# vilnik/incorporating-different-sources

Hardware: AMD Instinct MI355X
Metric: rolling windows/sec (higher is better)
Workload: dtype f64

## Files before the change

### incorporating_different_sources_amd/csrc/posterior_wave_impl.h

```cpp
#pragma once
#include <utility>

#include "posterior_fused_impl.h"

namespace {

template <int NT_, bool LEAN_ = true>
struct WCfg {
    static constexpr int NT = NT_;
    static constexpr int KP = 16 * NT;
    static constexpr int NTILES = NT * (NT + 1) / 2;
    static constexpr int MLD = 17;
    static constexpr int OFF_M = 0;
    static constexpr int OFF_DG = OFF_M + NT * 16 * MLD;
    static constexpr int OFF_IDT = OFF_DG + 256;
    static constexpr int OFF_VEC = OFF_IDT + 256;
    static constexpr int LDS_DOUBLES = OFF_VEC + KP;
    static constexpr int LDS_BYTES = LDS_DOUBLES * 8;
    static constexpr int OFF_SUB = LDS_DOUBLES;
};
constexpr int WAVE_LDS_LIMIT = 64 * 1024;
__host__ __device__ inline int wave_idx_rows(int n_r, int m, bool conj) {
    const int r = (conj && m > n_r) ? m : n_r;
    return (r + 63) & ~63;
}
__host__ __device__ inline int wave_idx_bytes(int n_r, int m, bool conj) { return wave_idx_rows(n_r, m, conj) * 12; }

constexpr int wtile(int NT, int I, int J) { return I * NT - I * (I - 1) / 2 + (J - I); }

template <int I, int J>
__device__ __forceinline__ void wave_post_tile(double* P, int k, int fr, int fq, const d4& t) {
    const int gj = 16 * J + fr;
#pragma unroll
    for (int r = 0; r < 4; ++r) {
        const int gi = 16 * I + fq + 4 * r;
        if (gi < k && gj < k && (I < J || gi <= gj)) {
            tp_post_store(P + (long long)gi * k + gj, t[r]);
            if (I < J || gi < gj) tp_post_store(P + (long long)gj * k + gi, t[r]);
        }
    }
}

template <int NT, int NWV>
constexpr int w2_owner(int J) {
    const int p = NT - 1 - J, g = p / NWV, i = p % NWV;
    return (g & 1) ? NWV - 1 - i : i;
}
template <int NT, int NWV>
constexpr int w2_count(int WV) {
    int n = 0;
    for (int J = 0; J < NT; ++J)
        if (w2_owner<NT, NWV>(J) == WV) n += J + 1;
    return n;
}
template <int NT, int NWV>
constexpr int w2_max_tiles() {
    int m = 0;
    for (int w = 0; w < NWV; ++w) m = w2_count<NT, NWV>(w) > m ? w2_count<NT, NWV>(w) : m;
    return m;
}
template <int NT, int NWV>
constexpr int w2_slot(int I, int J) {
    const int wv = w2_owner<NT, NWV>(J);
    int n = 0;
    for (int i = 0; i < NT; ++i)
        for (int j = i; j < NT; ++j) {
            if (i == I && j == J) return n;
            if (w2_owner<NT, NWV>(j) == wv) ++n;
        }
    return -1;
}
template <int NT, int NWV>
constexpr bool w2_owns_from(int WV, int I) {
    for (int J = I; J < NT; ++J)
        if (w2_owner<NT, NWV>(J) == WV) return true;
    return false;
}
template <int NT>
constexpr bool w2_one_wave_is_whole() {
    for (int J = 0; J < NT; ++J) {
        if (w2_owner<NT, 1>(J) != 0) return false;
        for (int I = 0; I <= J; ++I)
            if (w2_slot<NT, 1>(I, J) != wtile(NT, I, J)) return false;
    }
    return w2_count<NT, 1>(0) == NT * (NT + 1) / 2;
}
template <int... N>
constexpr bool w2_one_wave_is_whole_all(std::integer_sequence<int, N...>) { return (w2_one_wave_is_whole<N + 1>() && ...); }
static_assert(w2_one_wave_is_whole_all(std::make_integer_sequence<int, 15>{}),
              "w2_owner<NT,1>(J) == 0, w2_slot<NT,1>(I,J) == wtile(NT,I,J), w2_count<NT,1>(0) == NT(NT+1)/2 for NT = 1..15");

constexpr bool wave_tile_in_agpr(int t) { return t < 32; }

template <int T>
__device__ __forceinline__ void wave_mfma_agpr(d4& c, double a, double b) {
    if constexpr (wave_tile_in_agpr(T)) asm volatile("s_nop 1\n\tv_mfma_f64_16x16x4_f64 %0, %1, %2, %0" : "+a"(c) : "v"(a), "v"(b));
    else asm volatile("s_nop 1\n\tv_mfma_f64_16x16x4_f64 %0, %1, %2, %0" : "+v"(c) : "v"(a), "v"(b));
}
template <int T>
__device__ __forceinline__ void wave_settle1(d4& c0) {
    if constexpr (wave_tile_in_agpr(T)) asm volatile("s_nop 15\n\ts_nop 7" : "+a"(c0));
    else asm volatile("s_nop 15\n\ts_nop 7" : "+v"(c0));
}
template <int T>
__device__ __forceinline__ void wave_pin1(d4& c0) {
    if constexpr (wave_tile_in_agpr(T)) asm volatile("" : "+a"(c0));
    else asm volatile("" : "+v"(c0));
}
__device__ __forceinline__ void wave_settle14(d4& c0, d4& c1, d4& c2, d4& c3, d4& c4, d4& c5, d4& c6, d4& c7, d4& c8, d4& c9,
                                              d4& c10, d4& c11, d4& c12, d4& c13) {
    asm volatile("s_nop 15\n\ts_nop 7" : "+a"(c0), "+a"(c1), "+a"(c2), "+a"(c3), "+a"(c4), "+a"(c5), "+a"(c6), "+a"(c7), "+a"(c8),
                 "+a"(c9), "+a"(c10), "+a"(c11), "+a"(c12), "+a"(c13));
}
template <int N>
__device__ __forceinline__ void wave_pin(d4 (&acc)[N]) {
    static_for<0, N>([&](auto tc) __attribute__((always_inline)) { wave_pin1<decltype(tc)::value>(acc[decltype(tc)::value]); });
}
template <bool GROUPED, int N>
__device__ __forceinline__ void wave_settle(d4 (&acc)[N]) {
    if constexpr (GROUPED) {
        static_for<0, (N + 13) / 14>([&](auto gc) __attribute__((always_inline)) {
            constexpr int b = 14 * decltype(gc)::value;
            if constexpr (b + 14 <= N && wave_tile_in_agpr(b + 13)) {
                wave_settle14(acc[b], acc[b + 1], acc[b + 2], acc[b + 3], acc[b + 4], acc[b + 5], acc[b + 6], acc[b + 7], acc[b + 8],
                              acc[b + 9], acc[b + 10], acc[b + 11], acc[b + 12], acc[b + 13]);
            } else {
                static_for<b, (b + 14 < N ? b + 14 : N)>([&](auto tc) __attribute__((always_inline)) {
                    wave_settle1<decltype(tc)::value>(acc[decltype(tc)::value]);
                });
            }
        });
    } else {
        wave_settle1<0>(acc[0]);
        static_for<1, N>([&](auto tc) __attribute__((always_inline)) { wave_pin1<decltype(tc)::value>(acc[decltype(tc)::value]); });
    }
}

struct WRows {
    const double* base;
    long long ld;
    const int* ridx;
    long long first;
    const double* sub_row;
    int count;
    int count0;
    int jump;
    bool off32 = false;
};

template <int NT, int NWV, int WV, bool HF, bool LEAN>
__device__ __forceinline__ void wave_gram(const WRows& src, const long long (&coff)[NT], int k, int lane,
                                          double (&shift)[NT], double (&w0v)[NT], bool ones, bool lazy_mask,
                                          d4 (&acc)[w2_count<NT, NWV>(WV)], const int* lds_rows, const double* lds_sub,
                                          double (&csum)[NT], double& usum) {
    constexpr int kI = NT - 1;
    const int fr = lane & 15, fq = lane >> 4;
    const int kc = k - 16 * kI;
    const bool cvl = fr < kc;
    const double border = HF ? ((ones && fr == kc + 1) ? 1.0 : 0.0) : ((fr == kc) ? 1.0 : 0.0);
    const int nks = (src.count + 3) >> 2;
    const bool has_sub = !HF && src.sub_row != nullptr;

    int row_pref = 0;
    double sub_pref = 0.0;
    auto prefetch = [&](int ks) __attribute__((always_inline)) {
        int r = 4 * ks + fq;
        r = r < src.count ? r : src.count - 1;
        row_pref = lds_rows[r];
        if (has_sub) sub_pref = lds_sub[r];
    };
    if constexpr (!LEAN) prefetch(0);
    const char* ub = (const char*)(LEAN ? src.base + src.first * src.ld : src.base);
    const unsigned ld8 = (unsigned)src.ld * 8u;
    unsigned c8[NT];
#pragma unroll
    for (int i = 0; i < NT; ++i) c8[i] = 8u * (unsigned)coff[i];
    auto load = [&](double (&v)[NT], double& sub, int ks) __attribute__((always_inline)) {
        int r = 4 * ks + fq;
        r = r < src.count ? r : src.count - 1;
        if (LEAN || src.off32) {
            unsigned row;
            if constexpr (LEAN) row = (unsigned)(r + (r >= src.count0 ? src.jump : 0));
            else row = (unsigned)row_pref;
            if constexpr (LEAN) {
                const unsigned r0 = __umul24(row, ld8) + c8[0];
#pragma unroll
                for (int i = 0; i < NT - 1; ++i) v[i] = *(const double*)(ub + (size_t)r0 + 128 * i);
                v[NT - 1] = *(const double*)(ub + (size_t)(__umul24(row, ld8) + c8[NT - 1]));
            } else {
                const unsigned ro = __umul24(row, ld8);
#pragma unroll
                for (int i = 0; i < NT; ++i) v[i] = *(const double*)(ub + (size_t)(ro + c8[i]));
            }
        } else {
            const double* p = src.base + (long long)row_pref * src.ld;
#pragma unroll
            for (int i = 0; i < NT; ++i) v[i] = p[coff[i]];
        }
        sub = 0.0;
        if constexpr (!LEAN) {
            if (has_sub) sub = sub_pref;
            prefetch(ks + 1);
        } else {
            if (has_sub) sub = src.sub_row[r];
        }
    };
    auto step = [&](double (&v)[NT], double sub, int ks, auto maskc) __attribute__((always_inline)) {
        constexpr bool MASK = decltype(maskc)::value != 0;
        if (HF) {
#pragma unroll
            for (int i = 0; i < NT; ++i) v[i] -= shift[i];
        } else if (has_sub) {
#pragma unroll
            for (int i = 0; i < NT; ++i) v[i] -= sub;
        }
        v[kI] = cvl ? v[kI] : border;
        if (MASK) {
            const bool rv = 4 * ks + fq < src.count;
#pragma unroll
            for (int i = 0; i < NT; ++i) v[i] = rv ? v[i] : 0.0;
        }
        if (HF) {
            double z = 0.0;
#pragma unroll
            for (int i = 0; i < NT; ++i) z = fma(v[i], w0v[i], z);
            z = rowgroup_sum16(z);
            if (!ones) {
#pragma unroll
                for (int i = 0; i < NT; ++i) csum[i] += v[i];
                usum += z;
            }
            if (fr == kc) v[kI] = z;
        }
        static_for<0, NT>([&](auto Ic) __attribute__((always_inline)) {
            constexpr int I = decltype(Ic)::value;
            static_for<I, NT>([&](auto Jc) __attribute__((always_inline)) {
                constexpr int J = decltype(Jc)::value;
                if constexpr (w2_owner<NT, NWV>(J) == WV) {
                    constexpr int t = w2_slot<NT, NWV>(I, J);
                    wave_mfma_agpr<t>(acc[t], v[I], v[J]);
                }
            });
        });
    };

    if (nks <= 0) return;
    double va[NT], vb[NT], vc[NT];
    double sa = 0.0, sb = 0.0, sc = 0.0;
    load(va, sa, 0);
    load(vb, sb, 1);
    if (HF && lazy_mask) {
        __builtin_amdgcn_sched_barrier(0);
#pragma unroll
        for (int i = 0; i < NT; ++i) {
            const bool cv = 16 * i + fr < k;
            shift[i] = cv ? shift[i] : 0.0;
            w0v[i] = cv ? w0v[i] : 0.0;
        }
    }
    wave_pin(acc);
    int ks = 0;
#pragma nounroll
    for (; 4 * (ks + 3) <= src.count; ks += 3) {
        load(vc, sc, ks + 2);
        step(va, sa, ks, ic<0>{});
        load(va, sa, ks + 3);
        step(vb, sb, ks + 1, ic<0>{});
        load(vb, sb, ks + 4);
        step(vc, sc, ks + 2, ic<0>{});
    }
    if (ks < nks) {
        if (ks + 2 < nks) load(vc, sc, ks + 2);
        step(va, sa, ks, ic<1>{});
        if (ks + 1 < nks) step(vb, sb, ks + 1, ic<1>{});
        if (ks + 2 < nks) step(vc, sc, ks + 2, ic<1>{});
    }
    wave_settle<NWV == 1>(acc);
}

__device__ __forceinline__ void wave_stage_rows(const WRows& src, int lane, int* li, double* lsb) {
    for (int i = lane; i < src.count; i += 64) {
        li[i] = src.ridx ? src.ridx[i] : (int)(src.first + i);
        if (src.sub_row) lsb[i] = src.sub_row[i];
    }
    __builtin_amdgcn_fence(__ATOMIC_RELEASE, "wavefront");
    __builtin_amdgcn_wave_barrier();
}

template <int NT, bool LEAN, int MODE>
__device__ __forceinline__ void wave_window_body(const tp_kargs_t& A, double* lds) {
    constexpr bool FULL = MODE == 2;
    constexpr bool POST = MODE >= 3;
    constexpr int PLAIN = POST ? MODE - 3 : MODE;
    using C = WCfg<NT, LEAN>;
    const int lane = threadIdx.x;
    const int fr = lane & 15, fq = lane >> 4;
    const int k = A.k;
    __builtin_assume(k >= 16 * (NT - 1));
    __builtin_assume(k <= 16 * NT - 1);
    constexpr int kI = NT - 1;
    const int kc = k - 16 * kI;
    const int NTB = (kc == 0) ? NT - 1 : NT;
    const bool colv = fr < kc;
    const long long per_xcd = (A.w_count + 7) >> 3;
    const long long wl = (long long)(blockIdx.x & 7) * per_xcd + (blockIdx.x >> 3);
    if ((long long)(blockIdx.x >> 3) >= per_xcd || wl >= A.w_count) return;
    const long long w = A.w_first + wl;
    const int tid0 = lane;
    (void)tid0;

    const int* cols = (!LEAN && A.col_idx) ? A.col_idx + w * k : nullptr;
    long long coff[NT];
    if (cols != nullptr) {
        int cidx[NT];
#pragma unroll
        for (int i = 0; i < NT; ++i) {
            const int c = 16 * i + fr;
            cidx[i] = cols[c < k ? c : k - 1];
        }
#pragma unroll
        for (int i = 0; i < NT; ++i) coff[i] = (long long)cidx[i];
    } else {
#pragma unroll
        for (int i = 0; i < NT; ++i) {
            const int c = 16 * i + fr;
            coff[i] = (long long)(c < k ? c : k - 1);
        }
    }
    double* idx_sub_lds = LEAN ? nullptr : lds + C::OFF_SUB;
    int* idx_rows_lds = LEAN ? nullptr : (int*)(lds + C::OFF_SUB + wave_idx_rows(A.n_r, A.m, A.strategy == 0));
    d4 acc[C::NTILES];
    static_for<0, C::NTILES>([&](auto tc) __attribute__((always_inline)) { acc[decltype(tc)::value] = d4{0.0, 0.0, 0.0, 0.0}; });
    wave_pin(acc);

#pragma unroll
    for (int i = 0; i < 4; ++i) {
        const int e = lane + 64 * i;
        lds[C::OFF_IDT + e] = ((e >> 4) == (e & 15)) ? 1.0 : 0.0;
    }

    double n0 = 0.0, cc = 0.0, q0 = 0.0;
    const bool conj = PLAIN == 0 ? true : PLAIN == 1 ? false : (A.strategy == 0);
    const int dbg = (FULL && A.dbg_S1 != nullptr && w == A.dbg_w) ? A.dbg_mode : 0;

    auto dump_matrix = [&]() __attribute__((always_inline)) {
        static_for<0, NT>([&](auto Ic) __attribute__((always_inline)) {
            constexpr int I = decltype(Ic)::value;
            static_for<I, NT>([&](auto Jc) __attribute__((always_inline)) {
                constexpr int J = decltype(Jc)::value;
                constexpr int t = wtile(NT, I, J);
                const int gj = 16 * J + fr;
#pragma unroll
                for (int r = 0; r < 4; ++r) {
                    const int gi = 16 * I + fq + 4 * r;
                    if (gi < k && gj < k) {
                        A.dbg_S1[(long long)gi * k + gj] = acc[t][r];
                        A.dbg_S1[(long long)gj * k + gi] = acc[t][r];
                    }
                    if (gi < k && gj == k) A.dbg_S1[(long long)k * k + gi] = acc[t][r];
                }
            });
        });
    };
    auto corner = [&]() __attribute__((always_inline)) {
        constexpr int t = wtile(NT, kI, kI);
        const int ln = __builtin_amdgcn_readfirstlane(16 * (kc & 3) + kc);
        const double x0 = readlane_d(acc[t][0], ln), x1 = readlane_d(acc[t][1], ln);
        const double x2 = readlane_d(acc[t][2], ln), x3 = readlane_d(acc[t][3], ln);
        const int rr = kc >> 2;
        return rr == 0 ? x0 : rr == 1 ? x1 : rr == 2 ? x2 : x3;
    };

    TP_MARK(0);
    if (conj && dbg != 2) {
        n0 = A.n0[w];
        WRows hs;
        hs.base = A.hf_panel; hs.ld = A.hf_ld;
        hs.ridx = (!LEAN && A.hf_row_idx) ? A.hf_row_idx + w * (long long)A.m : nullptr;
        hs.first = A.hf_start ? A.hf_start[w] : 0;
        hs.sub_row = nullptr;
        hs.count = A.hf_count ? A.hf_count[w] : A.m;
        hs.count0 = 0x7fffffff; hs.jump = 0;
        hs.off32 = (A.hf_off32 & 1) != 0;
        const bool ones = kc < 15;
        double shift[NT], w0v[NT], csum[NT];
        double usum = 0.0;
        {
            const long long row0 = hs.ridx ? (long long)hs.ridx[0] : hs.first;
            const double* p0 = hs.base + row0 * (long long)hs.ld;
#pragma unroll
            for (int i = 0; i < NT; ++i) {
                const int c = 16 * i + fr;
                const int cl = c < k ? c : k - 1;
                const double sv = p0[coff[i]];
                const double wv = A.w0[w * k + cl];
                shift[i] = sv;
                w0v[i] = wv;
                csum[i] = 0.0;
            }
        }
        TP_MARK(1);
        const int hf_rows_all = hs.count;
        if (!hs.ridx) { hs.first += 1; hs.count -= 1; }
        else { hs.ridx += 1; hs.count -= 1; }
        if constexpr (!LEAN) wave_stage_rows(hs, lane, idx_rows_lds, idx_sub_lds);
        wave_gram<NT, 1, 0, true, LEAN>(hs, coff, k, lane, shift, w0v, ones, true, acc, idx_rows_lds, idx_sub_lds, csum, usum);
        hs.count = hf_rows_all;
        TP_MARK(2);
        const double invm = 1.0 / (double)hs.count;
        double tj[NT];
        double cz = corner();
        if (ones) {
            static_for<0, NT>([&](auto Ic) __attribute__((always_inline)) {
                constexpr int I = decltype(Ic)::value;
                constexpr int t = wtile(NT, I, kI);
                if (fr == kc + 1) {
#pragma unroll
                    for (int r = 0; r < 4; ++r)
                        lds[C::OFF_VEC + 16 * I + fq + 4 * r] = (I < kI || fq + 4 * r <= kc) ? acc[t][r] : 0.0;
                }
            });
        } else {
#pragma unroll
            for (int i = 0; i < NT; ++i) {
                double sc_ = csum[i];
                sc_ += __shfl_xor(sc_, 16, 64);
                sc_ += __shfl_xor(sc_, 32, 64);
                if (fq == 0) lds[C::OFF_VEC + 16 * i + fr] = (16 * i + fr < k) ? sc_ : 0.0;
            }
            double su = usum;
            su += __shfl_xor(su, 16, 64);
            su += __shfl_xor(su, 32, 64);
            __builtin_amdgcn_fence(__ATOMIC_RELEASE, "wavefront");
            __builtin_amdgcn_wave_barrier();
            if (lane == 0) lds[C::OFF_VEC + k] = su;
        }
        __builtin_amdgcn_fence(__ATOMIC_RELEASE, "wavefront");
        __builtin_amdgcn_wave_barrier();
#pragma unroll
        for (int J = 0; J < NT; ++J) tj[J] = lds[C::OFF_VEC + 16 * J + fr];
        {
            const double tk = lds[C::OFF_VEC + k];
            cz = fma(-(tk * invm), tk, cz);
        }
        const double mm = (double)hs.count;
        const double sc = n0 * (mm / (mm - 1.0));
        q0 = sc * cz;
        const double a = n0 + k + 2;
        cc = (2 * n0) / (a + sqrt(a * a + 4 * n0 * q0));
        const double fcol = colv ? sc : ((fr == kc) ? cc * sc : 0.0);
        static_for<0, NT>([&](auto Ic) __attribute__((always_inline)) {
            constexpr int I = decltype(Ic)::value;
            double ti[4];
#pragma unroll
            for (int r = 0; r < 4; ++r) ti[r] = -(lds[C::OFF_VEC + 16 * I + fq + 4 * r] * invm);
            static_for<I, NT>([&](auto Jc) __attribute__((always_inline)) {
                constexpr int J = decltype(Jc)::value;
                constexpr int t = wtile(NT, I, J);
                d4 x = acc[t];
#pragma unroll
                for (int r = 0; r < 4; ++r) x[r] = fma(ti[r], tj[J], x[r]);
                if constexpr (J < kI) {
                    x *= sc;
                } else if constexpr (I < kI) {
                    x *= fcol;
                } else {
#pragma unroll
                    for (int r = 0; r < 4; ++r) x[r] *= (fq + 4 * r < kc) ? fcol : 0.0;
                }
                acc[t] = x;
                wave_pin1<t>(acc[t]);
            });
            __builtin_amdgcn_sched_barrier(0);
        });
        __builtin_amdgcn_wave_barrier();
        if (dbg == 1) { dump_matrix(); return; }
    }
    TP_MARK(3);
    {
        WRows ds;
        ds.base = A.panel; ds.ld = A.panel_ld;
        ds.ridx = (!LEAN && A.row_idx) ? A.row_idx + w * (long long)A.n_r : nullptr;
        ds.first = A.start ? A.start[w] : 0;
        ds.sub_row = A.rf_adj ? A.rf_adj + w * (long long)A.n_r : nullptr;
        ds.count = A.n_rows ? A.n_rows[w] : A.n_r;
        ds.count0 = 0x7fffffff; ds.jump = 0;
        ds.off32 = (A.panel_off32 & 1) != 0;
        double none[NT] = {};
        bool shared = false;
        const double* q = nullptr;
        if constexpr (LEAN) {
            constexpr int BLK = 16;
            const long long b0 = (ds.first + BLK - 1) / BLK, b1 = (ds.first + ds.count) / BLK;
            const int Lw = (int)(b1 - b0);
            const int li = Lw == A.winsum_L[0] ? 0 : Lw == A.winsum_L[1] ? 1 : Lw == A.winsum_L[2] ? 2 : Lw == A.winsum_L[3] ? 3 : -1;
            shared = A.winsum != nullptr && Lw > 0 && li >= 0;
            if (shared) {
                ds.count0 = (int)(BLK * b0 - ds.first);
                ds.jump = (int)(BLK * b1 - ds.first) - ds.count0;
                ds.count = ds.count0 + (int)(ds.first + ds.count - BLK * b1);
                q = A.winsum + ((long long)li * A.prefix_nblk + b0) * ((long long)C::NTILES * 256);
            }
        }
        TP_MARK(32);
        typedef double d2 __attribute__((ext_vector_type(2)));
        constexpr int GRP = 7, NG = (C::NTILES + GRP - 1) / GRP;
        const d2* pq = (const d2*)q + lane;
        d2 qa[GRP][2], qb[GRP][2];
        auto qload = [&](d2 (&v2)[GRP][2], auto gc) __attribute__((always_inline)) {
            constexpr int g = decltype(gc)::value;
            static_for<0, GRP>([&](auto ec) __attribute__((always_inline)) {
                constexpr int e = decltype(ec)::value;
                constexpr int t = g * GRP + e;
                if constexpr (t < C::NTILES) {
                    v2[e][0] = pq[(long long)t * 128];
                    v2[e][1] = pq[(long long)t * 128 + 64];
                }
            });
        };
        auto qadd = [&](d2 (&v2)[GRP][2], auto gc) __attribute__((always_inline)) {
            constexpr int g = decltype(gc)::value;
            static_for<0, GRP>([&](auto ec) __attribute__((always_inline)) {
                constexpr int e = decltype(ec)::value;
                constexpr int t = g * GRP + e;
                if constexpr (t < C::NTILES) {
                    d4 x = acc[t];
                    x[0] += v2[e][0][0]; x[1] += v2[e][0][1];
                    x[2] += v2[e][1][0]; x[3] += v2[e][1][1];
                    acc[t] = x;
                    wave_pin1<t>(acc[t]);
                }
            });
        };
        if constexpr (!LEAN) wave_stage_rows(ds, lane, idx_rows_lds, idx_sub_lds);
        double nosum = 0.0;
        wave_gram<NT, 1, 0, false, LEAN>(ds, coff, k, lane, none, none, false, false, acc, idx_rows_lds, idx_sub_lds, none, nosum);
        TP_MARK(33);
        if (LEAN && shared) {
            qload(qa, ic<0>{});
            static_for<0, NG>([&](auto gc) __attribute__((always_inline)) {
                constexpr int g = decltype(gc)::value;
                if constexpr (g + 1 < NG) {
                    if constexpr (g % 2 == 0) qload(qb, ic<g + 1>{}); else qload(qa, ic<g + 1>{});
                }
                __builtin_amdgcn_sched_barrier(0);
                if constexpr (g % 2 == 0) qadd(qa, gc); else qadd(qb, gc);
                __builtin_amdgcn_sched_barrier(0);
            });
        }
    }
    TP_MARK(34);
    static_for<0, NT>([&](auto Ic) __attribute__((always_inline)) {
        constexpr int I = decltype(Ic)::value;
        constexpr int t = wtile(NT, I, kI);
        if constexpr (I == kI) {
            d4 x = acc[t];
#pragma unroll
            for (int r = 0; r < 4; ++r) x[r] = (fq + 4 * r >= kc) ? 0.0 : x[r];
            acc[t] = x;
            wave_pin1<t>(acc[t]);
        }
    });
    __builtin_amdgcn_sched_barrier(0);
    if (dbg == 2) { dump_matrix(); return; }

    if (!conj) {
        static_for<0, NT>([&](auto Ic) __attribute__((always_inline)) {
            constexpr int I = decltype(Ic)::value;
            constexpr int t = wtile(NT, I, kI);
            if (fr == kc) {
#pragma unroll
                for (int r = 0; r < 4; ++r) lds[C::OFF_VEC + 16 * I + fq + 4 * r] = acc[t][r];
            }
        });
        __builtin_amdgcn_fence(__ATOMIC_RELEASE, "wavefront");
        __builtin_amdgcn_wave_barrier();
        const double invN = !FULL ? 1.0 / (double)A.N : A.center_rows == 2 ? 0.0
                          : 1.0 / (double)(A.center_rows ? (A.n_rows ? A.n_rows[w] : A.n_r) : A.N);
        const double sh_d = (FULL && A.shift) ? A.shift[2 * w] : 0.0;
        const double sh_e = (FULL && A.shift) ? A.shift[2 * w + 1] : 0.0;
        double tj[NT];
#pragma unroll
        for (int J = 0; J < NT; ++J) tj[J] = lds[C::OFF_VEC + 16 * J + fr];
        static_for<0, NT>([&](auto Ic) __attribute__((always_inline)) {
            constexpr int I = decltype(Ic)::value;
            double ti[4];
#pragma unroll
            for (int r = 0; r < 4; ++r) ti[r] = lds[C::OFF_VEC + 16 * I + fq + 4 * r];
            static_for<I, NT>([&](auto Jc) __attribute__((always_inline)) {
                constexpr int J = decltype(Jc)::value;
                constexpr int t = wtile(NT, I, J);
                d4 x = acc[t];
#pragma unroll
                for (int r = 0; r < 4; ++r) {
                    const bool on = (J < kI || colv) && (I < kI || fq + 4 * r < kc);
                    const double add = sh_e + ((I == J && fq + 4 * r == fr) ? sh_d : 0.0);
                    x[r] += on ? add - invN * (ti[r] * tj[J]) : 0.0;
                }
                acc[t] = x;
                wave_pin1<t>(acc[t]);
            });
            __builtin_amdgcn_sched_barrier(0);
        });
        __builtin_amdgcn_wave_barrier();
    }
    if (FULL && A.rhs != nullptr) {
        static_for<0, NT>([&](auto Ic) __attribute__((always_inline)) {
            constexpr int I = decltype(Ic)::value;
            constexpr int t = wtile(NT, I, kI);
            if (fr == kc) {
#pragma unroll
                for (int r = 0; r < 4; ++r) {
                    const int gi = 16 * I + fq + 4 * r;
                    const int gl = gi < k ? gi : k - 1;
                    const double x = A.rhs[w * k + gl];
                    acc[t][r] = (gi < k) ? x : 0.0;
                }
            }
            wave_pin1<t>(acc[t]);
        });
    }
    if (FULL && A.out_rhs != nullptr) {
        static_for<0, NT>([&](auto Ic) __attribute__((always_inline)) {
            constexpr int I = decltype(Ic)::value;
            constexpr int t = wtile(NT, I, kI);
            if (fr == kc) {
#pragma unroll
                for (int r = 0; r < 4; ++r) {
                    const int gi = 16 * I + fq + 4 * r;
                    if (gi < k) A.out_rhs[w * k + gi] = acc[t][r];
                }
            }
        });
    }
    if (dbg == 3) dump_matrix();
    if constexpr (POST) {
        double* P = tp_post_window(A, w);
        if (P != nullptr) {
            static_for<0, NT>([&](auto Ic) __attribute__((always_inline)) {
                constexpr int I = decltype(Ic)::value;
                static_for<I, NT>([&](auto Jc) __attribute__((always_inline)) {
                    constexpr int J = decltype(Jc)::value;
                    wave_post_tile<I, J>(P, k, fr, fq, acc[wtile(NT, I, J)]);
                });
            });
        }
    }

    TP_MARK(4);
    double badacc = 0.0;
    static_for<0, NT>([&](auto jc) __attribute__((always_inline)) {
        constexpr int j = decltype(jc)::value;
        if (j < NTB) {
            const int npiv = (k - 16 * j < 16) ? (k - 16 * j) : 16;
            constexpr int tjj = wtile(NT, j, j);
#pragma unroll
            for (int r = 0; r < 4; ++r) lds[C::OFF_DG + (fq + 4 * r) * 16 + fr] = acc[tjj][r];
            __builtin_amdgcn_fence(__ATOMIC_RELEASE, "wavefront");
            __builtin_amdgcn_wave_barrier();
            const int c16 = lane & 15;
            double a[16];
            const double* src = (lane < 16) ? (lds + C::OFF_DG) : (lds + C::OFF_IDT);
#pragma unroll
            for (int i = 0; i < 16; ++i) a[i] = src[i * 16 + c16];
            constexpr bool ALL16 = j < kI;
            constexpr int RL = 2;
            typedef double d2 __attribute__((ext_vector_type(2)));
            double* const mrows = lds + C::OFF_DG;
            const int mw = (lane < 16) ? lane : 32 + lane;
            double d0 = readlane_d(a[0], 0);
            double rinv = rsqrt_cubic(d0);
#pragma unroll
            for (int p = 0; p < 16; ++p) {
                if (ALL16 || p < npiv) {
                    a[p] *= rinv;
                    badacc = fma(0.0, rinv, badacc);
                    const int i0 = p + 1 + RL;
                    double* const mrow = mrows + 16 * (p & 1);
                    if (i0 < 16) {
                        mrow[mw] = a[p];
                        __builtin_amdgcn_fence(__ATOMIC_RELEASE, "wavefront");
                        __builtin_amdgcn_wave_barrier();
                    }
                    double mm[16];
#pragma unroll
                    for (int i = i0; i < 16; ++i) {
                        if ((i & 1) == 0) {
                            const d2 v = *(const d2*)(mrow + i);
                            mm[i] = v[0];
                            mm[i + 1] = v[1];
                        } else if (i == i0) {
                            mm[i] = mrow[i];
                        }
                    }
                    double rinv_next = 1.0;
                    if (p + 1 < 16) {
                        double dn = fma(-a[p], a[p], a[p + 1]);
                        if (!ALL16) dn = (p + 1 < npiv) ? dn : 1.0;
                        rinv_next = readlane_d(rsqrt_cubic(dn), p + 1);
                    }
#pragma unroll
                    for (int i = p + 1; i < i0 && i < 16; ++i) {
                        const double sI = readlane_d(a[p], i);
                        a[i] = fma(-sI, a[p], a[i]);
                    }
#pragma unroll
                    for (int i = i0; i < 16; ++i) a[i] = fma(-mm[i], a[p], a[i]);
                    rinv = rinv_next;
                    __builtin_amdgcn_sched_barrier(0);
                }
            }
            if (lane >= 16 && lane < 32) {
#pragma unroll
                for (int i = 0; i < 16; ++i) lds[C::OFF_M + (j * 16 + i) * C::MLD + c16] = (i < npiv) ? a[i] : 0.0;
            }
            __builtin_amdgcn_fence(__ATOMIC_RELEASE, "wavefront");
            __builtin_amdgcn_wave_barrier();
            double mop[4];
#pragma unroll
            for (int r = 0; r < 4; ++r) mop[r] = lds[C::OFF_M + (j * 16 + fr) * C::MLD + 4 * r + fq];
            static_for<j, NT>([&](auto Jc) __attribute__((always_inline)) {
                constexpr int J = decltype(Jc)::value;
                if constexpr (J > j || j == kI) {
                    constexpr int t = wtile(NT, j, J);
                    d4 rj = d4{0.0, 0.0, 0.0, 0.0};
#pragma unroll
                    for (int r = 0; r < 4; ++r) rj = __builtin_amdgcn_mfma_f64_16x16x4f64(mop[r], acc[t][r], rj, 0, 0, 0);
                    acc[t] = rj;
                }
            });
            static_for<j + 1, NT>([&](auto Ic) __attribute__((always_inline)) {
                constexpr int I = decltype(Ic)::value;
                static_for<I, NT>([&](auto Jc) __attribute__((always_inline)) {
                    constexpr int J = decltype(Jc)::value;
                    constexpr int t = wtile(NT, I, J), tI = wtile(NT, j, I), tJ = wtile(NT, j, J);
#pragma unroll
                    for (int r = 0; r < 4; ++r)
                        acc[t] = __builtin_amdgcn_mfma_f64_16x16x4f64(acc[tI][r], acc[tJ][r], acc[t], 0, 0, 1);
                });
            });
        }
    });

    TP_MARK(5);
    double q1 = 0.0;
    double wcol[NT];
#pragma unroll
    for (int J = 0; J < NT; ++J) wcol[J] = 0.0;
    {
        double q1p = 0.0;
        static_for<0, NT>([&](auto Ic) __attribute__((always_inline)) {
            constexpr int I = decltype(Ic)::value;
            constexpr int t = wtile(NT, I, kI);
#pragma unroll
            for (int r = 0; r < 4; ++r) {
                const double y = (fr == kc && (I < kI || fq + 4 * r < kc)) ? acc[t][r] : 0.0;
                q1p = fma(y, y, q1p);
            }
        });
        q1 = wave_sum64(q1p);
    }
    static_for<0, NT>([&](auto ic) __attribute__((always_inline)) {
        constexpr int Ib = NT - 1 - decltype(ic)::value;
        if (Ib < NTB) {
            constexpr int tb = wtile(NT, Ib, kI);
            double z[4];
#pragma unroll
            for (int r = 0; r < 4; ++r) {
                double u = 0.0;
                static_for<Ib + 1, NT>([&](auto Jc) __attribute__((always_inline)) {
                    constexpr int J = decltype(Jc)::value;
                    constexpr int t = wtile(NT, Ib, J);
                    if (J < NTB) u = fma(acc[t][r], wcol[J], u);
                });
                const double y = (fr == kc && (Ib < kI || fq + 4 * r < kc)) ? acc[tb][r] : 0.0;
                z[r] = rowgroup_sum16(y - u);
            }
            d4 wt = d4{0.0, 0.0, 0.0, 0.0};
#pragma unroll
            for (int r = 0; r < 4; ++r) {
                const double mrow = lds[C::OFF_M + (Ib * 16 + 4 * r + fq) * C::MLD + fr];
                wt = __builtin_amdgcn_mfma_f64_16x16x4f64(z[r], mrow, wt, 0, 0, 0);
            }
            wcol[Ib] = wt[0];
            __builtin_amdgcn_sched_barrier(0);
        }
    });

    TP_MARK(6);
    {
        const double n1 = n0 + (double)A.N;
        const double denom = n1 - q1;
        bool nonfinite = false;
        static_for<0, NT>([&](auto Ic) __attribute__((always_inline)) {
            constexpr int I = decltype(Ic)::value;
            const int gi = 16 * I + fr;
            double out;
            if (conj) out = 1.0 / A.gamma * ((n1 + k + 2) * wcol[I] / denom);
            else out = 1.0 / A.gamma * wcol[I];
            if (fq == (I & 3) && gi < k) {
                A.weights[w * k + gi] = out;
                if (!isfinite(out)) nonfinite = true;
            }
        });
        const bool anybad = __any(nonfinite ? 1 : 0) != 0;
        const bool notpd = __any((badacc != badacc) ? 1 : 0) != 0;
        if (lane == 0) {
            int st = TP_KSTATUS_OK;
            if (notpd) st = TP_KSTATUS_NOT_PD;
            else if (anybad) st = TP_KSTATUS_NONFINITE;
            else if (conj && !(denom > 0.0)) st = TP_KSTATUS_BAD_DENOM;
            A.status[w] = st;
            if (A.aux) {
                double* ax = A.aux + w * 8;
                ax[0] = n0; ax[1] = conj ? n1 : 0.0; ax[2] = cc; ax[3] = q0; ax[4] = q1;
                ax[5] = conj ? denom : 0.0; ax[6] = 0.0; ax[7] = 0.0;
            }
        }
    }
    TP_MARK(7);
}

constexpr int wave_occupancy(int nt) { return nt <= 3 ? 4 : nt <= 5 ? 2 : 1; }

template <int NT, bool LEAN, int MODE>
__global__ void __launch_bounds__(64, wave_occupancy(NT)) posterior_wave_kernel(const tp_kargs_t A) {
    extern __shared__ __attribute__((aligned(16))) double lds[];
    wave_window_body<NT, LEAN, MODE>(A, lds);
}

template <int NT, bool LEAN>
inline int wave_lds_bytes(const tp_kargs_t& a) {
    return WCfg<NT, LEAN>::LDS_BYTES + (LEAN ? 0 : wave_idx_bytes(a.n_r, a.m, a.strategy == 0));
}

constexpr bool wave_post_built(int nt, bool lean, int mode) { return !(mode == 3 && nt == 8 && !lean); }

template <int NT, bool LEAN, int MODE>
hipError_t wave_launch_mode(const tp_kargs_t& a, int grid8, hipStream_t stream) {
    if constexpr (!wave_post_built(NT, LEAN, MODE)) {
        return hipErrorNotSupported;
    } else {
        const int lds_bytes = wave_lds_bytes<NT, LEAN>(a);
        if (lds_bytes > WAVE_LDS_LIMIT) return hipErrorNotSupported;
        static std::atomic<unsigned long long> attr_done{0};
        { hipError_t e = tp_allow_dynamic_lds(attr_done, posterior_wave_kernel<NT, LEAN, MODE>, WAVE_LDS_LIMIT); if (e != hipSuccess) return e; }
        hipLaunchKernelGGL((posterior_wave_kernel<NT, LEAN, MODE>), dim3(grid8), dim3(64), lds_bytes, stream, a);
        return hipGetLastError();
    }
}

template <int NT, bool LEAN>
hipError_t wave_launch_variant(const tp_kargs_t& a, int grid, hipStream_t stream, tp_launch_info_t* info) {
    if (info) { info->grid = grid; info->block = 64; info->lds_bytes = wave_lds_bytes<NT, LEAN>(a); info->ntile = NT; }
    const int grid8 = 8 * ((grid + 7) / 8);
    const int mode = wave_mode(a);
    switch (mode == 2 ? 2 : tp_post_mode(a, mode)) {
        case 0: return wave_launch_mode<NT, LEAN, 0>(a, grid8, stream);
        case 1: return wave_launch_mode<NT, LEAN, 1>(a, grid8, stream);
        case 3: return wave_launch_mode<NT, LEAN, 3>(a, grid8, stream);
        case 4: return wave_launch_mode<NT, LEAN, 4>(a, grid8, stream);
        default: return hipErrorNotSupported;
    }
}

}
```

Measured before the change: 17.95 million.

## Prefetch daily-pass rows and window scalars during high-frequency tile update

Window scalars (start, row counts, hf start/count, n0) are now loaded at the top of the kernel for small NT, and the daily-panel setup is computed before the high-frequency pass. For eligible configurations, the first two row loads of the daily Gram pass are issued after the first tile-row update of the high-frequency stage and handed into wave_gram. The aim is to hide global-load latency at the start of the daily pass behind the remaining high-frequency arithmetic. In exchange it raises register pressure, since extra row buffers stay live across the tile updates, and it adds aliasing reads through a spare pointer when the index arrays are absent.

```diff
diff --git a/incorporating_different_sources_amd/csrc/posterior_wave_impl.h b/incorporating_different_sources_amd/csrc/posterior_wave_impl.h
--- a/incorporating_different_sources_amd/csrc/posterior_wave_impl.h
+++ b/incorporating_different_sources_amd/csrc/posterior_wave_impl.h
@@ -148,11 +148,18 @@
     bool off32 = false;
 };
 
-template <int NT, int NWV, int WV, bool HF, bool LEAN>
+template <int NT>
+struct WaveRowsAhead {
+    double va[NT], vb[NT];
+    double sa, sb;
+};
+template <int NT, int NWV, int WV, bool HF, bool LEAN, class Pre = std::nullptr_t>
 __device__ __forceinline__ void wave_gram(const WRows& src, const long long (&coff)[NT], int k, int lane,
                                           double (&shift)[NT], double (&w0v)[NT], bool ones, bool lazy_mask,
                                           d4 (&acc)[w2_count<NT, NWV>(WV)], const int* lds_rows, const double* lds_sub,
-                                          double (&csum)[NT], double& usum) {
+                                          double (&csum)[NT], double& usum, Pre pre = nullptr) {
+    constexpr bool PRE = !std::is_same<Pre, std::nullptr_t>::value;
+    static_assert(!PRE || (LEAN && !HF), "rows requested ahead: contiguous daily pass only");
     constexpr int kI = NT - 1;
     const int fr = lane & 15, fq = lane >> 4;
     const int kc = k - 16 * kI;
@@ -247,8 +254,14 @@
     if (nks <= 0) return;
     double va[NT], vb[NT], vc[NT];
     double sa = 0.0, sb = 0.0, sc = 0.0;
-    load(va, sa, 0);
-    load(vb, sb, 1);
+    if constexpr (PRE) {
+#pragma unroll
+        for (int i = 0; i < NT; ++i) { va[i] = pre->va[i]; vb[i] = pre->vb[i]; }
+        sa = pre->sa; sb = pre->sb;
+    } else {
+        load(va, sa, 0);
+        load(vb, sb, 1);
+    }
     if (HF && lazy_mask) {
         __builtin_amdgcn_sched_barrier(0);
 #pragma unroll
@@ -277,6 +290,29 @@
     }
     wave_settle<NWV == 1>(acc);
 }
+
+template <int NT>
+__device__ __forceinline__ void wave_gram_request(const WRows& src, const long long (&coff)[NT], int lane, WaveRowsAhead<NT>& ah) {
+    const int fq = lane >> 4;
+    if (src.count <= 0) return;
+    const char* ub = (const char*)(src.base + src.first * src.ld);
+    const unsigned ld8 = (unsigned)src.ld * 8u;
+    auto load = [&](double (&v)[NT], double& sub, int ks) __attribute__((always_inline)) {
+        int r = 4 * ks + fq;
+        r = r < src.count ? r : src.count - 1;
+        const unsigned row = (unsigned)(r + (r >= src.count0 ? src.jump : 0));
+        const unsigned r0 = __umul24(row, ld8) + 8u * (unsigned)coff[0];
+#pragma unroll
+        for (int i = 0; i < NT - 1; ++i) v[i] = *(const double*)(ub + (size_t)r0 + 128 * i);
+        v[NT - 1] = *(const double*)(ub + (size_t)(__umul24(row, ld8) + 8u * (unsigned)coff[NT - 1]));
+        sub = src.sub_row != nullptr ? src.sub_row[r] : 0.0;
+    };
+    load(ah.va, ah.sa, 0);
+    load(ah.vb, ah.sb, 1);
+}
+
+constexpr bool wave_scalars_early(int nt) { return nt <= 8; }
+constexpr bool wave_rows_ahead(int nt, int mode) { return wave_scalars_early(nt) && !(nt == 8 && mode == 3); }
 
 __device__ __forceinline__ void wave_stage_rows(const WRows& src, int lane, int* li, double* lsb) {
     for (int i = lane; i < src.count; i += 64) {
@@ -371,15 +407,64 @@
         return rr == 0 ? x0 : rr == 1 ? x1 : rr == 2 ? x2 : x3;
     };
 
+    constexpr bool EARLY = LEAN && !FULL && wave_scalars_early(NT);
+    typedef long long ll_any __attribute__((may_alias));
+    typedef int int_any __attribute__((may_alias));
+    long long w_start = 0, w_hf_start = 0;
+    int w_rows = 0, w_hf_count = 0;
+    if constexpr (EARLY) {
+        const void* spare = A.panel;
+        w_start = *(const ll_any*)(A.start ? (const void*)(A.start + w) : spare);
+        w_rows = *(const int_any*)(A.n_rows ? (const void*)(A.n_rows + w) : spare);
+        if constexpr (PLAIN == 0) {
+            n0 = A.n0[w];
+            w_hf_start = *(const ll_any*)(A.hf_start ? (const void*)(A.hf_start + w) : spare);
+            w_hf_count = *(const int_any*)(A.hf_count ? (const void*)(A.hf_count + w) : spare);
+        }
+    }
+    WRows ds_a;
+    bool shared_a = false;
+    const double* q_a = nullptr;
+    auto daily_setup = [&](WRows& ds, bool& shared, const double*& q) __attribute__((always_inline)) {
+        ds.base = A.panel; ds.ld = A.panel_ld;
+        ds.ridx = (!LEAN && A.row_idx) ? A.row_idx + w * (long long)A.n_r : nullptr;
+        if constexpr (EARLY) ds.first = A.start ? w_start : 0;
+        else ds.first = A.start ? A.start[w] : 0;
+        ds.sub_row = A.rf_adj ? A.rf_adj + w * (long long)A.n_r : nullptr;
+        if constexpr (EARLY) ds.count = A.n_rows ? w_rows : A.n_r;
+        else ds.count = A.n_rows ? A.n_rows[w] : A.n_r;
+        ds.count0 = 0x7fffffff; ds.jump = 0;
+        ds.off32 = (A.panel_off32 & 1) != 0;
+        if constexpr (LEAN) {
+            constexpr int BLK = 16;
+            const long long b0 = (ds.first + BLK - 1) / BLK, b1 = (ds.first + ds.count) / BLK;
+            const int Lw = (int)(b1 - b0);
+            const int li = Lw == A.winsum_L[0] ? 0 : Lw == A.winsum_L[1] ? 1 : Lw == A.winsum_L[2] ? 2 : Lw == A.winsum_L[3] ? 3 : -1;
+            shared = A.winsum != nullptr && Lw > 0 && li >= 0;
+            if (shared) {
+                ds.count0 = (int)(BLK * b0 - ds.first);
+                ds.jump = (int)(BLK * b1 - ds.first) - ds.count0;
+                ds.count = ds.count0 + (int)(ds.first + ds.count - BLK * b1);
+                q = A.winsum + ((long long)li * A.prefix_nblk + b0) * ((long long)C::NTILES * 256);
+            }
+        }
+    };
+    WaveRowsAhead<NT> ahead;
+    (void)ahead;
+    constexpr bool AHEAD = LEAN && PLAIN == 0 && wave_rows_ahead(NT, MODE);
+
     TP_MARK(0);
+    if constexpr (EARLY) daily_setup(ds_a, shared_a, q_a);
     if (conj && dbg != 2) {
-        n0 = A.n0[w];
+        if constexpr (!EARLY) n0 = A.n0[w];
         WRows hs;
         hs.base = A.hf_panel; hs.ld = A.hf_ld;
         hs.ridx = (!LEAN && A.hf_row_idx) ? A.hf_row_idx + w * (long long)A.m : nullptr;
-        hs.first = A.hf_start ? A.hf_start[w] : 0;
+        if constexpr (EARLY) hs.first = A.hf_start ? w_hf_start : 0;
+        else hs.first = A.hf_start ? A.hf_start[w] : 0;
         hs.sub_row = nullptr;
-        hs.count = A.hf_count ? A.hf_count[w] : A.m;
+        if constexpr (EARLY) hs.count = A.hf_count ? w_hf_count : A.m;
+        else hs.count = A.hf_count ? A.hf_count[w] : A.m;
         hs.count0 = 0x7fffffff; hs.jump = 0;
         hs.off32 = (A.hf_off32 & 1) != 0;
         const bool ones = kc < 15;
@@ -449,7 +534,7 @@
         const double a = n0 + k + 2;
         cc = (2 * n0) / (a + sqrt(a * a + 4 * n0 * q0));
         const double fcol = colv ? sc : ((fr == kc) ? cc * sc : 0.0);
-        static_for<0, NT>([&](auto Ic) __attribute__((always_inline)) {
+        auto tile_row = [&](auto Ic) __attribute__((always_inline)) {
             constexpr int I = decltype(Ic)::value;
             double ti[4];
 #pragma unroll
@@ -472,36 +557,28 @@
                 wave_pin1<t>(acc[t]);
             });
             __builtin_amdgcn_sched_barrier(0);
-        });
+        };
+        if constexpr (AHEAD) {
+            static_for<0, 1>(tile_row);
+            wave_gram_request<NT>(ds_a, coff, lane, ahead);
+            __builtin_amdgcn_sched_barrier(0);
+            static_for<1, NT>(tile_row);
+        } else {
+            static_for<0, NT>(tile_row);
+        }
         __builtin_amdgcn_wave_barrier();
         if (dbg == 1) { dump_matrix(); return; }
     }
     TP_MARK(3);
     {
-        WRows ds;
-        ds.base = A.panel; ds.ld = A.panel_ld;
-        ds.ridx = (!LEAN && A.row_idx) ? A.row_idx + w * (long long)A.n_r : nullptr;
-        ds.first = A.start ? A.start[w] : 0;
-        ds.sub_row = A.rf_adj ? A.rf_adj + w * (long long)A.n_r : nullptr;
-        ds.count = A.n_rows ? A.n_rows[w] : A.n_r;
-        ds.count0 = 0x7fffffff; ds.jump = 0;
-        ds.off32 = (A.panel_off32 & 1) != 0;
+        WRows ds_d;
+        bool shared_d = false;
+        const double* q_d = nullptr;
+        if constexpr (!EARLY) daily_setup(ds_d, shared_d, q_d);
+        WRows& ds = EARLY ? ds_a : ds_d;
+        const bool shared = EARLY ? shared_a : shared_d;
+        const double* q = EARLY ? q_a : q_d;
         double none[NT] = {};
-        bool shared = false;
-        const double* q = nullptr;
-        if constexpr (LEAN) {
-            constexpr int BLK = 16;
-            const long long b0 = (ds.first + BLK - 1) / BLK, b1 = (ds.first + ds.count) / BLK;
-            const int Lw = (int)(b1 - b0);
-            const int li = Lw == A.winsum_L[0] ? 0 : Lw == A.winsum_L[1] ? 1 : Lw == A.winsum_L[2] ? 2 : Lw == A.winsum_L[3] ? 3 : -1;
-            shared = A.winsum != nullptr && Lw > 0 && li >= 0;
-            if (shared) {
-                ds.count0 = (int)(BLK * b0 - ds.first);
-                ds.jump = (int)(BLK * b1 - ds.first) - ds.count0;
-                ds.count = ds.count0 + (int)(ds.first + ds.count - BLK * b1);
-                q = A.winsum + ((long long)li * A.prefix_nblk + b0) * ((long long)C::NTILES * 256);
-            }
-        }
         TP_MARK(32);
         typedef double d2 __attribute__((ext_vector_type(2)));
         constexpr int GRP = 7, NG = (C::NTILES + GRP - 1) / GRP;
@@ -534,7 +611,10 @@
         };
         if constexpr (!LEAN) wave_stage_rows(ds, lane, idx_rows_lds, idx_sub_lds);
         double nosum = 0.0;
-        wave_gram<NT, 1, 0, false, LEAN>(ds, coff, k, lane, none, none, false, false, acc, idx_rows_lds, idx_sub_lds, none, nosum);
+        if constexpr (AHEAD)
+            wave_gram<NT, 1, 0, false, LEAN>(ds, coff, k, lane, none, none, false, false, acc, idx_rows_lds, idx_sub_lds, none, nosum, &ahead);
+        else
+            wave_gram<NT, 1, 0, false, LEAN>(ds, coff, k, lane, none, none, false, false, acc, idx_rows_lds, idx_sub_lds, none, nosum);
         TP_MARK(33);
         if (LEAN && shared) {
             qload(qa, ic<0>{});
```

Measured after the change: 18.08 million, median of 6. No clear change (+0.7%).
